# jianwang-mpi/GlobalEgoMocap

Hardware: AMD Instinct MI355X
Metric: optimised windows/sec (10-frame, 15-joint) (higher is better)
Workload: dtype f32

## Files before the change

__graft_entry__.py:

```python
import os
import subprocess
import sys

ROOT = os.path.dirname(os.path.abspath(__file__))
if ROOT not in sys.path:
    sys.path.insert(0, ROOT)

CSRC = os.path.join(ROOT, "globalegomocap_amd", "csrc")
LIB_DIR = os.path.join(ROOT, "globalegomocap_amd", "_lib")
LIB = os.path.join(LIB_DIR, "libgem_hip.so")
SOURCES = ["gem_api.hip", "weights.hip", "stage.hip", "gemm_f32.hip", "gemm_bf16.hip", "decoder_bf16.hip", "energy.hip", "lbfgs.hip", "tail.hip", "tail_bf16.hip", "train.hip", "errors.hip", "chunk_io.hip"]


def _stale():
    if not os.path.exists(LIB):
        return True
    t = os.path.getmtime(LIB)
    deps = [os.path.join(CSRC, f) for f in os.listdir(CSRC)] + [os.path.join(ROOT, "include", "gem_hip.h"),
                                                                os.path.abspath(__file__)]
    return any(os.path.getmtime(d) > t for d in deps)


NO_PACKED_FP32 = ["-Xclang", "-target-feature", "-Xclang", "-packed-fp32-ops", "-DGEM_NO_PACKED_FP32"]
FP_CONTRACT = ["-ffp-contract=on"]
EXTRA_FLAGS = {}
OBJ_DIR = os.path.join(ROOT, "build", "obj")


def _compile_one(args):
    hipcc, src, obj, extra = args
    cmd = [hipcc, "--offload-arch=gfx950", "-O3", "-std=c++17", "-fPIC", "-c", "-Wall", "-Wno-unused-function"] + NO_PACKED_FP32 + FP_CONTRACT + extra + ["-o", obj, src]
    r = subprocess.run(cmd, stderr=subprocess.PIPE, text=True)
    rest = [l for l in r.stderr.splitlines() if "'-packed-fp32-ops' is not a recognized feature for this target" not in l]
    if rest:
        sys.stderr.write("\n".join(rest) + "\n")
    if r.returncode:
        raise subprocess.CalledProcessError(r.returncode, cmd)
    return obj


def _objdump(hipcc=None):
    import shutil
    roots = [os.environ.get("ROCM_PATH", "/opt/rocm")]
    if hipcc:
        roots.insert(0, os.path.dirname(os.path.dirname(os.path.realpath(hipcc))))
    for r in roots:
        c = os.path.join(r, "lib", "llvm", "bin", "llvm-objdump")
        if os.path.exists(c):
            return c
    c = shutil.which("llvm-objdump")
    if c:
        return c
    raise RuntimeError("llvm-objdump not found (looked under %s and on PATH): the build cannot prove the library free of packed "
                       "fp32 arithmetic and refuses to ship it unchecked" % ", ".join(roots))


def device_isa(lib=None, hipcc=None):
    import glob
    import shutil
    import tempfile
    lib = lib or LIB
    objdump = _objdump(hipcc)
    tmp = tempfile.mkdtemp(prefix="gem_isa_")
    try:
        local = os.path.join(tmp, "lib.so")
        shutil.copy(lib, local)
        subprocess.run([objdump, "--offloading", local], check=True, cwd=tmp, stdout=subprocess.DEVNULL, stderr=subprocess.DEVNULL)
        parts = sorted(glob.glob(local + ".*gfx950*"))
        if not parts:
            raise RuntimeError("no gfx950 code object found in %s" % lib)
        return "\n".join(subprocess.run([objdump, "-d", p], check=True, capture_output=True, text=True).stdout for p in parts)
    finally:
        shutil.rmtree(tmp, ignore_errors=True)


def check_no_packed_fp32(lib=None, hipcc=None):
    import re
    isa = device_isa(lib, hipcc)
    bad = re.findall(r"^.*\bv_pk_(?:fma|mul|add)_f32\b.*$", isa, flags=re.M)
    if bad:
        raise RuntimeError("%d packed fp32 VALU instructions in %s (gfx950 hazard beside bf16 MFMAs, DESIGN.md section 4), e.g. %s"
                           % (len(bad), lib or LIB, bad[0].strip()))
    return isa.count("\n")


def build(force=False):
    os.makedirs(LIB_DIR, exist_ok=True)
    if force or _stale():
        from concurrent.futures import ThreadPoolExecutor
        hipcc = os.environ.get("HIPCC", "/opt/rocm/bin/hipcc")
        os.makedirs(OBJ_DIR, exist_ok=True)
        headers = [os.path.join(CSRC, f) for f in os.listdir(CSRC) if f.endswith(".h")] + [os.path.join(ROOT, "include", "gem_hip.h"),
                                                                                             os.path.abspath(__file__)]
        newest_header = max(os.path.getmtime(hd) for hd in headers)
        jobs, objs = [], []
        for s in SOURCES:
            src, obj = os.path.join(CSRC, s), os.path.join(OBJ_DIR, s.replace(".hip", ".o"))
            objs.append(obj)
            if force or not os.path.exists(obj) or os.path.getmtime(obj) < max(os.path.getmtime(src), newest_header):
                jobs.append((hipcc, src, obj, EXTRA_FLAGS.get(s, [])))
        with ThreadPoolExecutor(max_workers=min(6, max(1, len(jobs)))) as pool:
            list(pool.map(_compile_one, jobs))
        tmp_lib = LIB + ".unchecked.%d" % os.getpid()
        try:
            subprocess.run([hipcc, "--offload-arch=gfx950", "-fPIC", "-shared", "-o", tmp_lib] + objs, check=True)
            check_no_packed_fp32(tmp_lib, hipcc)
            os.replace(tmp_lib, LIB)
        finally:
            if os.path.exists(tmp_lib):
                os.remove(tmp_lib)
    import globalegomocap_amd
    from globalegomocap_amd import _capi
    _capi.load_library()


def smoke():
    build()
    import numpy as np
    import torch
    from globalegomocap_amd import synth, vae as vae_schema
    from globalegomocap_amd.camera import FisheyeCamera, DEFAULT_CALIBRATION
    from globalegomocap_amd.engine import WindowEngine, energy_weights, LOCAL_STAGE
    from oracle import np_oracle as O

    torch.cuda.set_device(0)
    shape = vae_schema.VAEShape(latent_dim=64, hidden=(16, 16, 32, 32, 64))
    sd = vae_schema.synthetic_state_dict(shape, seed=3, gain=2.0)
    cam = FisheyeCamera.from_json(DEFAULT_CALIBRATION)
    seq = synth.make_sequence(n_frames=100, seed=4, camera=cam)
    est = np.asarray(seq["estimated_local_skeleton"], dtype=np.float32)
    heat = np.asarray(seq["heatmap_list"], dtype=np.float32)
    starts = np.arange(0, 91, 8, dtype=np.int32)
    nw = len(starts)
    pose = np.stack([est[s:s + 10] for s in starts])
    eng = WindowEngine(shape, cam, max_windows=16)
    eng.load_vae(LOCAL_STAGE, sd)
    mb = eng.mean_bone_length(est)
    rng = np.random.default_rng(0)
    z = rng.normal(size=(nw, shape.latent_dim)).astype(np.float32)
    w = energy_weights(1e-2, 1e-2, 1e-1, 1e-3, 1e-2)
    E, parts, dz, X = eng.energy_grad(LOCAL_STAGE, z, pose, mb, w, heat, starts)
    torch.cuda.synchronize()
    vae = O.fold_vae(sd)
    ocam = O.Camera(poly=np.asarray(cam.poly_w2c), cx=cam.cx, cy=cam.cy)
    ow = O.Weights(1e-2, 1e-2, 1e-1, 1e-3, 1e-2)
    mb_o = O.mean_bone_length(est)
    assert np.allclose(mb.cpu().numpy(), mb_o, rtol=1e-5, atol=1e-6)
    for b in range(nw):
        Xo, acts = O.decode(vae, z[b:b + 1], keep=True)
        f, p, dX = O.energy_and_grad(Xo[0], pose[b], mb_o, ow, ocam, heat[starts[b]:starts[b] + 10])
        dzo = O.decode_backward(vae, dX[None], acts)[0]
        assert np.allclose(X[b].cpu().numpy(), Xo[0], rtol=1e-4, atol=1e-5), "decode mismatch"
        assert abs(float(E[b]) - f) <= 1e-5 * abs(f) + 1e-7, ("energy mismatch", float(E[b]), f)
        assert np.abs(dz[b].cpu().numpy() - dzo).max() <= 1e-3 * np.abs(dzo).max() + 1e-7, "gradient mismatch"
    eps = rng.normal(size=(nw, shape.latent_dim)).astype(np.float32)
    out, stats = eng.optimize_stage(LOCAL_STAGE, pose, mb, eps, w, heat, starts)
    torch.cuda.synchronize()
    st = stats.cpu().numpy()
    assert (st[:, 3] == 1).all(), "a window did not finish"
    trace = eng.read_trace(nw)
    final = np.ascontiguousarray(st[:, 2]).view(np.float32)
    errs, self_errs = [], []
    for b in range(nw):
        X0 = pose[b].astype(np.float32)
        z0 = O.latent_from_pose(vae, X0.reshape(1, 10, 45), eps[b].reshape(1, -1))[0]
        losses = []

        def fun(zz):
            Xd, acts = O.decode(vae, zz[None], keep=True)
            f, _, dX = O.energy_and_grad(Xd[0], X0, mb_o, ow, ocam, heat[starts[b]:starts[b] + 10])
            losses.append(f)
            return f, O.decode_backward(vae, dX[None], acts)[0]
        zo, so = O.lbfgs_strong_wolfe(fun, z0, None)
        ref = O.decode(vae, zo[None])[0]
        n_ref = len(losses)
        zp, _ = O.lbfgs_strong_wolfe(fun, z0 + 1e-6 * np.sign(z0), None)
        self_errs.append(float(np.linalg.norm(O.decode(vae, zp[None])[0] - ref, axis=-1).mean()))
        losses = losses[:n_ref]
# ... 20 lines not shown
```

globalegomocap_amd/csrc/gem_internal.h:

```cpp
#pragma once
#if defined(__HIP_DEVICE_COMPILE__) && !defined(GEM_NO_PACKED_FP32)
#error "compile with: -Xclang -target-feature -Xclang -packed-fp32-ops -DGEM_NO_PACKED_FP32 (__graft_entry__.NO_PACKED_FP32)"
#endif

#include <hip/hip_runtime.h>
#include <stdint.h>
#include <atomic>
#include <set>
#include <string>
#include <vector>

#include "../../include/gem_hip.h"

namespace gem {

constexpr int PAD = 64;
constexpr float LEAKY_SLOPE = 0.01f;
constexpr double BN_EPS = 1e-5;
constexpr int MAX_HIST = 128;
constexpr int MAXJ_ERR = GEM_MAX_JOINTS;
constexpr int N_LOG = 1 << 16;
constexpr int TRACE_ROUNDS = 64;

inline int pad64(int x) { return (x + PAD - 1) / PAD * PAD; }
// ... 172 lines not shown
    v += dpp_move<0xB1>(v);
    v += dpp_move<0x4E>(v);
    v += dpp_move<0x141>(v);
    v += dpp_move<0x140>(v);
    return ((read_lane(v, 0) + read_lane(v, 16)) + read_lane(v, 32)) + read_lane(v, 48);
}
__device__ __forceinline__ double wave_max_dpp(double v) {
    v = nan_max(v, dpp_move<0xB1>(v));
    v = nan_max(v, dpp_move<0x4E>(v));
    v = nan_max(v, dpp_move<0x141>(v));
    v = nan_max(v, dpp_move<0x140>(v));
    return nan_max(nan_max(nan_max(read_lane(v, 0), read_lane(v, 16)), read_lane(v, 32)), read_lane(v, 48));
}

}

namespace gem {
struct GraphKey {
    int kind = 0, stage = 0, B = 0, precision = 0;
    bool tex_cache = true;
    const void* ptr[12] = {};
    gem_energy_weights w[2] = {};
    gem_lbfgs_opts opt = {};
    void* stream = nullptr;
};
struct GraphEntry {
    GraphKey key;
    hipGraph_t graph = nullptr;
    hipGraphExec_t exec = nullptr;
    uint64_t last_use = 0;
};
}

struct gem_handle {
    gem_config cfg;
    int T, J, C, Cp, D, Dp, top, topp;
    gem::StageNet net[2];
    gem::Workspace ws;
    gem::Profile prof;
    int precision = 0;
    int n_cu = 256;
    double* post_work = nullptr;
    size_t post_work_elems = 0;
    bool tex_cache = true;
    bool graphs_on = false;
    std::vector<gem::GraphEntry> graphs;
    uint64_t graph_tick = 0;
    int64_t graph_replays = 0, graph_captures = 0;
    int* d_parents = nullptr;
    int* d_children = nullptr;
};

namespace gem {

void note_kernel(gem_handle* h, const void* host_fn);
inline void commit_kernel_names(gem_handle* h, int family) {
    if (family >= 0 && family < 4) h->prof.names[family].insert(h->prof.pending.begin(), h->prof.pending.end());
    h->prof.pending.clear();
}

int launch_gemm(gem_handle* h, const Layer& L, int epi, const float* A, int lda, const float* aux, float* Cout, int ldc,
                int M, int T, hipStream_t s, int family, const GemmOpts& o = GemmOpts());

int pick_splitk(const gem_handle* h, long blocks, int n_tiles, size_t slab_elems);

struct DynSplit { int RT, SK, per; size_t slab; };
__host__ __device__ inline DynSplit dyn_split(int M, int BM, int CT, int W, int n_tiles, int ldc) {
    DynSplit d;
    d.RT = (M + BM - 1) / BM;
    if (d.RT < 1) d.RT = 1;
    int cap = W / (d.RT * CT);
    if (cap < 1) cap = 1;
    int mx = n_tiles / 4;
    if (mx < 1) mx = 1;
    const int sk = cap < mx ? cap : mx;
    d.per = (n_tiles + sk - 1) / sk;
    d.SK = (n_tiles + d.per - 1) / d.per;
    d.slab = (size_t)d.RT * BM * ldc;
    return d;
}
__device__ inline void slab_layout(const SlabSrc& s, int& nslab, size_t& stride) {
    nslab = s.nslab;
    stride = s.stride;
    if (s.dyn_W > 0) {
        const DynSplit d = dyn_split(*s.m_dev, 64, s.CT, s.dyn_W, s.n_tiles, s.ldc);
        nslab = d.SK;
        stride = d.slab;
    }
}
bool rows_can_fuse_compaction(const gem_handle* h, const Layer& L, int lda, int ldc, int B, bool slabs);
int launch_splitk_reduce(gem_handle* h, int epi, int nslab, size_t slab, const float* bias, const float* aux, float* C, int M, int N,
                         int ldc, const int* m_dev, hipStream_t s, int dyn_W = 0, int n_tiles = 0);
int launch_gemm_bf16(gem_handle* h, const Layer& L, int epi, int nprod, const float* A, int lda, const float* aux, float* Cout,
                     int ldc, int M, int T, hipStream_t s, const GemmOpts& o);

enum Narrow {
    NARROW_BATCHED = 0,
    NARROW_TAIL_F32 = 1,
    NARROW_TAIL_BF16 = 2
};
struct Route {
    int precision = 0;
    Narrow narrow = NARROW_BATCHED;
    bool front = false;
    int tail_wgs = 0;
    int tail_cap = 0;
    Repack repack = REPACK_KERNEL;
};
enum Call { CALL_DECODE = 0, CALL_EVALUATE = 1, CALL_ROUNDS = 2 };
Route plan_route(const gem_handle* h, int stage, int B, Call call);

struct EnergyArgs;
int evaluate_bf16(gem_handle* h, const Route& rt, int stage, int B, const EnergyArgs& ea, hipStream_t s, bool forward_only, const RoundSet* rs,
                  SlabSrc* grad);
int launch_f32_to_bf16(const float* src, uint16_t* dst, size_t n, hipStream_t s);
int launch_f32_split_bf16(const float* src, uint16_t* hi, uint16_t* lo, size_t n, hipStream_t s);

int launch_pack_pose(const float* src, float* dst, int rows, int C, hipStream_t s);
int launch_unpack_pose(const float* src, float* dst, int rows, int C, hipStream_t s);
int launch_reparam(const float* mulv, const float* eps, float* mu, float* logvar, float* z, float* z2, int B, int D, int Dp,
                   hipStream_t s);
int launch_pad_latent(const float* z, float* zp, int B, int D, int Dp, hipStream_t s);
int launch_unpad_latent(const float* zp, float* z, int B, int D, int Dp, hipStream_t s);

struct EnergyArgs {
    const float* Xp;
    const float* X0;
    const float* heat;
    const int32_t* frame0;
    const float* mean_bone;
    float* dXp;
    uint16_t* dXp_b;
    double* f;
    double* parts;
    float w3d, ws, wb, wv, wr;
    double dw3d, dws, dwb, dwv, dwr;
    int T, J, H, W, n_poly;
    float poly[GEM_MAX_POLY];
    float cx, cy;
    const int* parents;
    const int* children;
    int* tex_key;
    float* tex_val;
    const int* n_dev;
    const int* perm;
};
int launch_energy(gem_handle* h, const EnergyArgs& a, int B, hipStream_t s);

constexpr int TAIL_MAX_LAYERS = 6;
struct TailLayerDev { const float* w4; const float* bias; int K, N; };
struct TailArgs {
    int n, B, G, forward_only, escr, mask_first;
    int waves, rows;
    SlabSrc in_slab;
    const float* in_bias;
    int in_bias_ld;
    long long* dbg_ts;
    TailLayerDev fwd[TAIL_MAX_LAYERS], bwd[TAIL_MAX_LAYERS];
    const float* a_in;
    float* g_out;
    uint16_t* g_out_b;
    float* Xp;
    int off_act[TAIL_MAX_LAYERS + 1], ld_act[TAIL_MAX_LAYERS + 1], off_g[2], ld_g, off_red, off_escr, off_zero, off_pre;
    EnergyArgs e;
};
size_t plan_tail(const std::vector<Layer>& dec, int start, int T, int J, TailArgs* out, bool shared = false);
void fill_tail_args(const gem_handle* h, const StageNet& net, const Route& rt, int B, bool forward_only, const SlabSrc& in_slab,
                    const EnergyArgs& ea, const RoundSet* rs, TailArgs* ta);
size_t plan_tail_for(const gem_handle* h, const std::vector<Layer>& dec, int start, int wgs, TailArgs* out);

constexpr int TB_MAX_LAYERS = 6;
struct TailB16Layer { int K, N; const float* bias; };
struct TailB16Args {
    int n, B, G, nrt, forward_only, mask_first;
    SlabSrc in_slab;
    const float* in_bias;
    int in_bias_ld;
    const uint16_t* a_in_b;
    uint16_t* g_out_b;
    float* Xp;
    long long* dbg_ts;
    const uint16_t* wstream;
    int steps_f, steps_total;
    TailB16Layer fwd[TB_MAX_LAYERS], bwd[TB_MAX_LAYERS];
    int off_act[TB_MAX_LAYERS + 1], ld_act[TB_MAX_LAYERS + 1];
    int off_mask[TB_MAX_LAYERS], ld_mask[TB_MAX_LAYERS];
    int off_x, escr, off_mb, off_zero, off_tab;
    int off_bwin, off_epair;
    EnergyArgs e;
};
size_t plan_tail_bf16(const std::vector<Layer>& dec, int start, int T, int J, TailB16Args* out, int nrt = 5);
int tail_bf16_row_tiles(const gem_handle* h, int B, int T);
int build_tail_bf16_stream(gem_handle* h, StageNet& net);
int launch_tail_bf16(gem_handle* h, const TailB16Args& a, size_t lds_bytes, hipStream_t s, const RoundSet* rs = nullptr);
int launch_tail(gem_handle* h, const TailArgs& a, size_t lds_bytes, hipStream_t s, const RoundSet* rs = nullptr);
int tail_cap_workgroups(const gem_handle* h, const std::vector<Layer>& dec, int start);
int launch_mean_bone(gem_handle* h, const float* pose, int n_frames, float* out, hipStream_t s);
int launch_gather_windows(const float* frames, const int32_t* frame0, float* out, int B, int T, int JC, hipStream_t s);
int launch_relative_global(const float* local, const double* cams, const int32_t* frame0, float* rel, int B, int T, int J,
                           hipStream_t s);
int launch_to_global(const float* rel, const double* cams, const int32_t* frame0, double* out, int B, int T, int J,
                     hipStream_t s);

int launch_errors(gem_handle* h, const double* est, const double* mid, const double* opt, const double* gt, int F,
                  const double* bone_mm, double* frame_out, double* out, hipStream_t s, int n_seq);
int launch_merge(const double* win, double* tmp, double* out, int n_chunks, int wpc, int T, int JC, int overlap, int smooth,
                 hipStream_t s);
size_t errors_frame_lds_bytes(int J);
void drop_graphs(gem_handle* h);
int post_scratch(gem_handle* h, size_t elems);
int launch_lift(gem_handle* h, const float* heat, const double* depth, int F, const double* poly, int n_poly, int up, int pad_x,
                int pad_y, double* out64, float* out32, hipStream_t s);

int launch_lbfgs_init(gem_handle* h, int B, hipStream_t s);
int launch_lbfgs_advance(gem_handle* h, int B, const gem_lbfgs_opts& o, const RoundSet& rs, const SlabSrc& grad, hipStream_t s);
int launch_lbfgs_stats(gem_handle* h, int B, gem_window_stats* out, hipStream_t s);
int launch_compact(gem_handle* h, const RoundSet& rs, int B, int force_all, hipStream_t s, int zero_after = 0);
int launch_lbfgs_debug_read(gem_handle* h, int B, gem_lbfgs_debug_state* out, float* x, float* d, float* trial, hipStream_t s);


}
```

globalegomocap_amd/csrc/tail.hip:

```cpp
#include <algorithm>

#include "energy_device.h"

namespace gem {

typedef float f32x16 __attribute__((ext_vector_type(16)));
typedef float f32x4 __attribute__((ext_vector_type(4)));

__device__ __forceinline__ float bf16_round(float x) {
    const __bf16 b = (__bf16)x;
    return (float)b;
}

constexpr int TAIL_WAVES = 8;
constexpr int TAIL_THREADS = TAIL_WAVES * 64;
constexpr int TAIL_WAVES_SHARED = 4;

constexpr int TAIL_ROWS = 16;

template <int W>
__device__ __forceinline__ void tail_prefetch_first(const TailLayerDev L, f32x4 (&dst)[4]) {
    const int lane = threadIdx.x & 63, wave = __builtin_amdgcn_readfirstlane(threadIdx.x >> 6);
    const int c = lane & 15, q = lane >> 4;
    const int n0 = wave * 16;
    if (n0 >= L.N) return;
    const f32x4* p = reinterpret_cast<const f32x4*>(L.w4) + (size_t)q * L.N + n0 + c;
#pragma unroll
    for (int g = 0; g < 4; ++g) dst[g] = p[(size_t)(4 * g) * L.N];
}

template <int W, int NT, typename Epi>
__device__ __forceinline__ void tail_gemm_nt(const float* in, int ld_in, const float* zero_line, const TailLayerDev L,
                                             const TailLayerDev next, bool has_next, int T, int R, f32x4 (&bpre)[4], Epi epi,
                                             int c0 = 0, bool use_pre = true) {
    const int tid = threadIdx.x, lane = tid & 63, wave = __builtin_amdgcn_readfirstlane(tid >> 6);
    const int fr = lane & 15, fq = lane >> 4;
    const int kb = L.K / 64, nblk = 3 * kb;
    const f32x4* W4 = reinterpret_cast<const f32x4*>(L.w4);
    constexpr int TS = 16 * W;
    const int n0 = wave * 16 + c0;
    if (n0 >= L.N) {
        if (has_next) tail_prefetch_first<W>(next, bpre);
        return;
    }
    const int row = fr;
    const int t_row = row % T;
    const bool row_ok = row < R;
    float bv[NT];
    f32x4 acc[NT];
#pragma unroll
    for (int i = 0; i < NT; ++i) {
        bv[i] = L.bias ? L.bias[n0 + TS * i + fr] : 0.f;
        acc[i] = f32x4{0.f, 0.f, 0.f, 0.f};
    }
    const f32x4* pB = W4 + (size_t)fq * L.N + n0 + fr;
    const int strideB = 16 * L.N;
    const int a_own = row * ld_in + 4 * fq;
    const int a_zero = (int)(zero_line - in) + 4 * fq;
    const bool ok_m = row_ok && t_row >= 1, ok_p = row_ok && t_row + 1 < T;
#define TAIL_LOAD_B(blk_, dst_)                                                                        \
    {                                                                                                  \
        const f32x4* p_ = pB + (size_t)(blk_) * strideB;                                               \
        _Pragma("unroll") for (int i = 0; i < NT; ++i)                                                 \
            _Pragma("unroll") for (int g = 0; g < 4; ++g) dst_[i][g] = p_[(size_t)(4 * g) * L.N + TS * i]; \
    }
#define TAIL_LOAD_A(blk_, dst_)                                                                        \
    {                                                                                                  \
        const int tap_ = ((blk_) >= kb) + ((blk_) >= 2 * kb), k0_ = ((blk_) - tap_ * kb) * 64;         \
        const bool ok_ = tap_ == 0 ? ok_m : (tap_ == 1 ? row_ok : ok_p);                               \
        const float* arow_ = in + (ok_ ? a_own + (tap_ - 1) * ld_in + k0_ : a_zero);                   \
        _Pragma("unroll") for (int g = 0; g < 4; ++g) dst_[g] = *reinterpret_cast<const f32x4*>(arow_ + 16 * g); \
    }
#define TAIL_COMPUTE(a_, b_)                                                                           \
    {                                                                                                  \
        _Pragma("unroll") for (int g = 0; g < 4; ++g) {                                                \
            _Pragma("unroll") for (int i = 0; i < NT; ++i) acc[i] = __builtin_amdgcn_mfma_f32_16x16x4f32(a_[g].x, b_[i][g].x, acc[i], 0, 0, 0); \
            _Pragma("unroll") for (int i = 0; i < NT; ++i) acc[i] = __builtin_amdgcn_mfma_f32_16x16x4f32(a_[g].y, b_[i][g].y, acc[i], 0, 0, 0); \
            _Pragma("unroll") for (int i = 0; i < NT; ++i) acc[i] = __builtin_amdgcn_mfma_f32_16x16x4f32(a_[g].z, b_[i][g].z, acc[i], 0, 0, 0); \
            _Pragma("unroll") for (int i = 0; i < NT; ++i) acc[i] = __builtin_amdgcn_mfma_f32_16x16x4f32(a_[g].w, b_[i][g].w, acc[i], 0, 0, 0); \
        }                                                                                              \
    }
    f32x4 b0[NT][4], b1[NT][4], a0[4], a1[4];
    TAIL_LOAD_B(0, b0);
    if (use_pre) {
#pragma unroll
        for (int g = 0; g < 4; ++g) b0[0][g] = bpre[g];
    }
    TAIL_LOAD_A(0, a0);
    const int npairs = nblk / 2;
#define TAIL_INTERLEAVE()                                                                                          \
    {                                                                                                              \
        _Pragma("unroll") for (int i_ = 0; i_ < 4 * NT; ++i_) { __builtin_amdgcn_sched_group_barrier(0x008, 2, 0); __builtin_amdgcn_sched_group_barrier(0x020, 1, 0); } \
        _Pragma("unroll") for (int i_ = 0; i_ < 4; ++i_) { __builtin_amdgcn_sched_group_barrier(0x008, 2 * NT, 0); __builtin_amdgcn_sched_group_barrier(0x100, 1, 0); } \
    }
    for (int p = 0; p < npairs; ++p) {
        const int blk = 2 * p;
        TAIL_LOAD_B(blk + 1, b1);
        TAIL_LOAD_A(blk + 1, a1);
        TAIL_COMPUTE(a0, b0);
        TAIL_INTERLEAVE();
        __builtin_amdgcn_sched_barrier(0);
        const int nxt = min(blk + 2, nblk - 1);
        TAIL_LOAD_B(nxt, b0);
        TAIL_LOAD_A(nxt, a0);
        TAIL_COMPUTE(a1, b1);
        TAIL_INTERLEAVE();
        __builtin_amdgcn_sched_barrier(0);
    }
#undef TAIL_INTERLEAVE
    if (nblk & 1) TAIL_COMPUTE(a0, b0);
    if (has_next) tail_prefetch_first<W>(next, bpre);
#undef TAIL_LOAD_A
#undef TAIL_LOAD_B
#undef TAIL_COMPUTE
#pragma unroll
    for (int i = 0; i < NT; ++i) epi(acc[i], 4 * fq, n0 + TS * i + fr, bv[i]);
}

template <int W, typename Epi>
__device__ __forceinline__ void tail_gemm(const float* in, int ld_in, const float* zero_line, const TailLayerDev L,
                                          const TailLayerDev next, bool has_next, int T, int R, f32x4 (&bpre)[4], Epi epi) {
    if constexpr (W == TAIL_WAVES_SHARED) {
        if (L.N > 32 * W) {
            tail_gemm_nt<W, 2>(in, ld_in, zero_line, L, next, false, T, R, bpre, epi);
            tail_gemm_nt<W, 2>(in, ld_in, zero_line, L, next, has_next, T, R, bpre, epi, 32 * W, false);
        } else if (L.N > 16 * W) tail_gemm_nt<W, 2>(in, ld_in, zero_line, L, next, has_next, T, R, bpre, epi);
        else tail_gemm_nt<W, 1>(in, ld_in, zero_line, L, next, has_next, T, R, bpre, epi);
    } else {
        if (L.N > 32 * W) tail_gemm_nt<W, 4>(in, ld_in, zero_line, L, next, has_next, T, R, bpre, epi);
        else if (L.N > 16 * W) tail_gemm_nt<W, 2>(in, ld_in, zero_line, L, next, has_next, T, R, bpre, epi);
        else tail_gemm_nt<W, 1>(in, ld_in, zero_line, L, next, has_next, T, R, bpre, epi);
    }
}

template <int NL, int W>
__global__ __launch_bounds__(64 * W, W == TAIL_WAVES_SHARED ? 3 : 2) void decoder_tail_kernel(TailArgs a) {
    constexpr int THREADS = 64 * W;
    constexpr bool TIGHT = W == TAIL_WAVES_SHARED;
    constexpr int STAGE_U = 2048 / THREADS;
    constexpr int PRE_E = TAIL_THREADS / THREADS;
    extern __shared__ __attribute__((aligned(16))) float lds[];
    const int tid = threadIdx.x, lane = tid & 63, wave = __builtin_amdgcn_readfirstlane(tid >> 6);
    const int T = a.e.T;
    int probe = 0;
#define TAIL_PROBE()                                                                                   \
    if (a.dbg_ts && blockIdx.x == 0 && tid == 0) {                                                     \
        a.dbg_ts[2 * probe] = clock64();                                                               \
        a.dbg_ts[2 * probe + 1] = wall_clock64();                                                      \
        ++probe;                                                                                       \
    }
    const int w0 = blockIdx.x * a.G;
    const int B = a.e.n_dev ? *a.e.n_dev : a.B;
    if (w0 >= B) return;
    const int nwin = min(a.G, B - w0);
    const int R = nwin * T;
    const size_t row0 = (size_t)w0 * T;

    {
        const int K0 = a.fwd[0].K, q4 = K0 / 4, n4 = (TIGHT ? a.rows : TAIL_ROWS) * q4;
        float* dst = lds + a.off_act[0];
        if (a.in_slab.base) {
            int nslab;
            size_t stride;
            slab_layout(a.in_slab, nslab, stride);
            for (int u = 0; u < STAGE_U; ++u) {
                const int i = tid + u * THREADS, r = i / q4, c = (i - r * q4) * 4;
                if (i >= n4) break;
                f32x4 v = {0.f, 0.f, 0.f, 0.f};
                if (r < R) {
                    const float* p = a.in_slab.base + (row0 + r) * K0 + c;
                    for (int z0 = 0; z0 < nslab; z0 += 8) {
                        f32x4 t[8];
#pragma unroll
                        for (int k = 0; k < 8; ++k) t[k] = *reinterpret_cast<const f32x4*>(p + (size_t)min(z0 + k, nslab - 1) * stride);
#pragma unroll
                        for (int k = 0; k < 8; ++k)
                            if (z0 + k < nslab) v += t[k];
                    }
                    v += *reinterpret_cast<const f32x4*>(a.in_bias + (r % T) * a.in_bias_ld + c);
#pragma unroll
                    for (int q = 0; q < 4; ++q) v[q] = v[q] > 0.f ? v[q] : v[q] * LEAKY_SLOPE;
                }
                *reinterpret_cast<f32x4*>(dst + r * a.ld_act[0] + c) = v;
            }
        } else {
            f32x4 v[STAGE_U];
#pragma unroll
            for (int u = 0; u < STAGE_U; ++u) {
                const int i = tid + u * THREADS, r = i / q4, c = (i - r * q4) * 4;
                v[u] = f32x4{0.f, 0.f, 0.f, 0.f};
                if (i < n4 && r < R) v[u] = *reinterpret_cast<const f32x4*>(a.a_in + (row0 + r) * K0 + c);
            }
#pragma unroll
            for (int u = 0; u < STAGE_U; ++u) {
                const int i = tid + u * THREADS, r = i / q4, c = (i - r * q4) * 4;
                if (i < n4) *reinterpret_cast<f32x4*>(dst + r * a.ld_act[0] + c) = v[u];
            }
        }
        if (tid < 64) lds[a.off_zero + tid] = 0.f;
    }
    float pre_x0[PRE_E], pre_mb = 0.f;
    int pre_par = 0, pre_ch[PRE_E];
#pragma unroll
    for (int k = 0; k < PRE_E; ++k) { pre_x0[k] = 0.f; pre_ch[k] = -1; }
    static_assert(MAXJ * MAXJ <= TAIL_THREADS && MAXJ <= 64, "the children table is parked by PRE_E passes of the workgroup");
    const bool pre_on = a.G == 1 && !a.forward_only && T * a.e.J * 3 <= TAIL_THREADS;
    if (pre_on) {
        const int J = a.e.J, n = T * J * 3, bw = a.e.perm ? a.e.perm[w0] : w0;
#pragma unroll
        for (int k = 0; k < PRE_E; ++k) {
            const int e = tid + k * THREADS;
            if (e < n) pre_x0[k] = a.e.X0[(size_t)bw * n + e];
            if (e < J * MAXJ) pre_ch[k] = a.e.children[e];
        }
        if (tid < J) { pre_mb = a.e.mean_bone[(size_t)bw * J + tid]; pre_par = a.e.parents[tid]; }
    }
    TAIL_PROBE();
    __syncthreads();
    TAIL_PROBE();

    f32x4 bpre[4];
    tail_prefetch_first<W>(a.fwd[0], bpre);
#pragma unroll
    for (int i = 0; i < NL; ++i) {
        const bool last = (i + 1 == NL);
        float* out = lds + a.off_act[i + 1];
        const int ldo = a.ld_act[i + 1];
        float* Xp = last ? a.Xp : nullptr;
        const TailLayerDev nxt = !last ? a.fwd[i + 1 < NL ? i + 1 : i] : a.bwd[NL - 1];
        tail_gemm<W>(lds + a.off_act[i], a.ld_act[i], lds + a.off_zero, a.fwd[i], nxt, !last || !a.forward_only, T, R, bpre,
                  [&](const f32x4& acc, int r0, int col, float bv) {
#pragma unroll
                      for (int e = 0; e < 4; ++e) {
                          float v = acc[e] + bv;
                          if (!last) v = v > 0.f ? v : v * LEAKY_SLOPE;
                          if (!TIGHT || r0 + e < a.rows) out[(r0 + e) * ldo + col] = v;
                          if (Xp && r0 + e < R) Xp[(row0 + r0 + e) * PAD + col] = v;
                      }
                  });
        if (i == 0 && pre_on) {
            const int J = a.e.J, n = T * J * 3;
            float* pre = lds + a.off_pre;
            int* prei = reinterpret_cast<int*>(pre + n + J);
#pragma unroll
            for (int k = 0; k < PRE_E; ++k) {
                const int e = tid + k * THREADS;
                if (e < n) pre[e] = pre_x0[k];
                if (e < J * MAXJ) prei[J + e] = pre_ch[k];
            }
            if (tid < J) { pre[n + tid] = pre_mb; prei[tid] = pre_par; }
        }
        __syncthreads();
        TAIL_PROBE();
    }
    if (a.forward_only) return;

    float* g_cur = lds + a.off_g[0];
    float* g_nxt = lds + a.off_g[1];
    if (a.G == 1) {
        float* scr = lds + a.off_escr;
        const int J = a.e.J, n = T * J * 3;
        const float* pre = lds + a.off_pre;
        const int* prei = reinterpret_cast<const int*>(pre + n + J);
        if (T == 10 && J == 15)
            energy_window<true, THREADS, 10, 15>(a.e, a.e.perm ? a.e.perm[w0] : w0, tid, lds + a.off_act[NL], a.ld_act[NL], scr,
                                                      scr + a.escr, scr + 2 * a.escr, scr + 3 * a.escr, g_cur, a.ld_g, a.fwd[NL - 1].N,
                                                      nullptr, pre_on ? pre : nullptr, pre_on ? pre + n : nullptr, pre_on ? prei : nullptr,
                                                      pre_on ? prei + J : nullptr);
        else
            energy_window<true, THREADS>(a.e, a.e.perm ? a.e.perm[w0] : w0, tid, lds + a.off_act[NL], a.ld_act[NL], scr,
                                              scr + a.escr, scr + 2 * a.escr, scr + 3 * a.escr, g_cur, a.ld_g, a.fwd[NL - 1].N,
                                              nullptr, pre_on ? pre : nullptr, pre_on ? pre + n : nullptr, pre_on ? prei : nullptr,
                                              pre_on ? prei + J : nullptr);
    } else if (wave < nwin) {
        float* scr = lds + a.off_escr + wave * 4 * a.escr;
        energy_window<false>(a.e, a.e.perm ? a.e.perm[w0 + wave] : w0 + wave, lane,
                             lds + a.off_act[NL] + wave * T * a.ld_act[NL], a.ld_act[NL], scr, scr + a.escr,
                             scr + 2 * a.escr, scr + 3 * a.escr, g_cur + wave * T * a.ld_g, a.ld_g, a.fwd[NL - 1].N);
    }
    __syncthreads();
    TAIL_PROBE();

#pragma unroll
    for (int i = NL - 1; i >= 0; --i) {
        const float* act = lds + a.off_act[i];
        const int lda = a.ld_act[i];
        const int ldg = a.ld_g;
        float* gout = a.g_out;
        uint16_t* gout_b = a.g_out_b;
        const int K0 = a.fwd[0].K;
        tail_gemm<W>(g_cur, a.ld_g, lds + a.off_zero, a.bwd[i], a.bwd[i > 0 ? i - 1 : 0], i > 0, T, R, bpre,
                  [&](const f32x4& acc, int r0, int col, float) {
#pragma unroll
                      for (int e = 0; e < 4; ++e) {
                          const int row = r0 + e;
                          const float v = (i > 0 || a.mask_first) ? acc[e] * (act[row * lda + col] > 0.f ? 1.f : LEAKY_SLOPE) : acc[e];
                          if (i > 0) { if (!TIGHT || row < a.rows) g_nxt[row * ldg + col] = v; }
                          else if (row < R) {
                              if (gout_b) gout_b[(row0 + row) * K0 + col] = (uint16_t)(__builtin_bit_cast(unsigned int, bf16_round(v)) >> 16);
                              else gout[(row0 + row) * K0 + col] = v;
                          }
                      }
                  });
        __syncthreads();
        TAIL_PROBE();
        float* t = g_cur; g_cur = g_nxt; g_nxt = t;
    }
#undef TAIL_PROBE
}

size_t plan_tail(const std::vector<Layer>& dec, int start, int T, int J, TailArgs* out, bool shared) {
    const int n = (int)dec.size() - start;
    if (start < 0 || n < 1 || n > TAIL_MAX_LAYERS || T > TAIL_ROWS) return 0;
    for (int i = start; i < (int)dec.size(); ++i) {
        const int K = dec[i].K, N = dec[i].N;
        auto ok = [](int v) { return v == 64 || v == 128 || v == 256 || v == 512; };
        if (!ok(K) || !ok(N)) return 0;
    }
    TailArgs a{};
    a.n = n;
    a.mask_first = start > 0;
    a.G = TAIL_ROWS / T;
    if (shared && a.G != 1) return 0;
    a.waves = shared ? TAIL_WAVES_SHARED : TAIL_WAVES;
    a.rows = shared ? a.G * T : TAIL_ROWS;
    const int rows = a.rows;
    int off = 0, maxg = 0;
    for (int i = 0; i <= n; ++i) {
        const int width = i == 0 ? dec[start].K : dec[start + i - 1].N;
        a.off_act[i] = off;
        a.ld_act[i] = width + 4;
        off += rows * (width + 4);
        if (i >= 1 && width > maxg) maxg = width;
    }
    a.ld_g = maxg + 4;
    a.off_g[0] = off; off += rows * a.ld_g;
    a.off_g[1] = off; off += rows * a.ld_g;
    a.escr = (T * J * 3 + 3) / 4 * 4;
    a.off_red = off;
    a.off_escr = off;
    off += a.G * 4 * a.escr;
    a.off_zero = off;
    off += 64;
    a.off_pre = off;
    if (a.G == 1) off += (T * J * 3 + 2 * J + J * MAXJ + 3) / 4 * 4;
    if (out) *out = a;
    return (size_t)off * sizeof(float);
}

template <int NL, int W>
static void launch_tail_as(gem_handle* h, const TailArgs& a, int wgs, size_t lds_bytes, hipStream_t s) {
    note_kernel(h, reinterpret_cast<const void*>(decoder_tail_kernel<NL, W>));
    hipLaunchKernelGGL((decoder_tail_kernel<NL, W>), dim3(wgs), dim3(64 * W), lds_bytes, s, a);
}

template <int W>
static int launch_tail_w(gem_handle* h, const TailArgs& a, int wgs, size_t lds_bytes, hipStream_t s) {
    switch (a.n) {
        case 1: launch_tail_as<1, W>(h, a, wgs, lds_bytes, s); break;
        case 2: launch_tail_as<2, W>(h, a, wgs, lds_bytes, s); break;
        case 3: launch_tail_as<3, W>(h, a, wgs, lds_bytes, s); break;
        case 4: launch_tail_as<4, W>(h, a, wgs, lds_bytes, s); break;
        case 5: launch_tail_as<5, W>(h, a, wgs, lds_bytes, s); break;
        case 6: launch_tail_as<6, W>(h, a, wgs, lds_bytes, s); break;
        default: set_error("launch_tail: unsupported number of fused layers"); return 1;
    }
    return 0;
}

static bool tail_can_share_cu(const std::vector<Layer>& dec, int start, int T, int J) {
    const size_t bytes = plan_tail(dec, start, T, J, nullptr, true);
    if (!bytes || 3 * bytes > 160 * 1024) return false;
    for (int i = start; i < (int)dec.size(); ++i)
        if (dec[i].N > 64 * TAIL_WAVES_SHARED || dec[i].K > 64 * TAIL_WAVES_SHARED) return false;
    return true;
}

size_t plan_tail_for(const gem_handle* h, const std::vector<Layer>& dec, int start, int wgs, TailArgs* out) {
    bool shared = wgs > h->n_cu && tail_can_share_cu(dec, start, h->T, h->J);
    if (const char* f = dev_env("GEM_TAIL_WAVES")) shared = atoi(f) == TAIL_WAVES_SHARED && tail_can_share_cu(dec, start, h->T, h->J);
    return plan_tail(dec, start, h->T, h->J, out, shared);
}

int tail_cap_workgroups(const gem_handle* h, const std::vector<Layer>& dec, int start) {
    if (const char* f = dev_env("GEM_TAIL_CAP")) return atoi(f) * h->n_cu;
    return (tail_can_share_cu(dec, start, h->T, h->J) ? 10 : 5) * h->n_cu;
}

int launch_tail(gem_handle* h, const TailArgs& a, size_t lds_bytes, hipStream_t s, const RoundSet* rs) {
    static PerDeviceOnce attr_once;
    if (attr_once.need(h->cfg.device)) {
        const void* ks[] = {reinterpret_cast<const void*>(decoder_tail_kernel<1, 8>), reinterpret_cast<const void*>(decoder_tail_kernel<2, 8>),
                            reinterpret_cast<const void*>(decoder_tail_kernel<3, 8>), reinterpret_cast<const void*>(decoder_tail_kernel<4, 8>),
                            reinterpret_cast<const void*>(decoder_tail_kernel<5, 8>), reinterpret_cast<const void*>(decoder_tail_kernel<6, 8>),
                            reinterpret_cast<const void*>(decoder_tail_kernel<1, 4>), reinterpret_cast<const void*>(decoder_tail_kernel<2, 4>),
                            reinterpret_cast<const void*>(decoder_tail_kernel<3, 4>), reinterpret_cast<const void*>(decoder_tail_kernel<4, 4>),
                            reinterpret_cast<const void*>(decoder_tail_kernel<5, 4>), reinterpret_cast<const void*>(decoder_tail_kernel<6, 4>)};
        for (const void* k : ks) GEM_HIP(hipFuncSetAttribute(k, hipFuncAttributeMaxDynamicSharedMemorySize, 160 * 1024));
    }
    Profile::Rec rec;
    const bool prof = h->prof.on;
    if (prof) {
        GEM_HIP(hipEventCreate(&rec.a)); GEM_HIP(hipEventCreate(&rec.b));
        rec.family = 1;
        double per_window = 0.0;
        for (int i = 0; i < a.n; ++i) per_window += 2.0 * 3.0 * a.fwd[i].K * a.fwd[i].N * a.e.T;
        if (!a.forward_only) per_window *= 2.0;
        rec.flops = per_window * a.B;
        if (rs) { rec.log_idx = rs->log_idx; rec.flops_per_window = per_window; }
        GEM_HIP(hipEventRecord(rec.a, s));
    }
    const int wgs = (a.B + a.G - 1) / a.G;
    if (a.waves != TAIL_WAVES && a.waves != TAIL_WAVES_SHARED) { set_error("launch_tail: the arguments do not come from plan_tail"); return 1; }
    if (a.waves == TAIL_WAVES_SHARED ? launch_tail_w<TAIL_WAVES_SHARED>(h, a, wgs, lds_bytes, s) : launch_tail_w<TAIL_WAVES>(h, a, wgs, lds_bytes, s))
        return 1;
    GEM_HIP(hipGetLastError());
    if (prof) { GEM_HIP(hipEventRecord(rec.b, s)); h->prof.recs.push_back(rec); }
    commit_kernel_names(h, prof ? 1 : -1);
    return 0;
}

}
```

Before: 32070.

## Deepen tail GEMM weight prefetch with register ring and early next-layer prefetch

The fused decoder-tail GEMM's two-buffer ping-pong becomes a configurable register ring. When the tail layers are narrow (at most two column tiles), the kernel prefetches the next layer's B blocks and bias for every tile before computing the current layer, so those global loads overlap the current MFMA work. Kernels are now also specialised on the widest layer, so narrow networks drop the four-tile path and its register pressure, and a higher unroll threshold is set for tail.hip. The cost is more live registers and more code paths, which can lower occupancy or cause spills.

```diff
diff --git a/__graft_entry__.py b/__graft_entry__.py
--- a/__graft_entry__.py
+++ b/__graft_entry__.py
@@ -23,7 +23,7 @@
 
 NO_PACKED_FP32 = ["-Xclang", "-target-feature", "-Xclang", "-packed-fp32-ops", "-DGEM_NO_PACKED_FP32"]
 FP_CONTRACT = ["-ffp-contract=on"]
-EXTRA_FLAGS = {}
+EXTRA_FLAGS = {"tail.hip": ["-mllvm", "-pragma-unroll-threshold=65536"]}
 OBJ_DIR = os.path.join(ROOT, "build", "obj")
 
 
diff --git a/globalegomocap_amd/csrc/gem_internal.h b/globalegomocap_amd/csrc/gem_internal.h
--- a/globalegomocap_amd/csrc/gem_internal.h
+++ b/globalegomocap_amd/csrc/gem_internal.h
@@ -348,6 +348,7 @@
 struct TailArgs {
     int n, B, G, forward_only, escr, mask_first;
     int waves, rows;
+    int maxnt;
     SlabSrc in_slab;
     const float* in_bias;
     int in_bias_ld;
diff --git a/globalegomocap_amd/csrc/tail.hip b/globalegomocap_amd/csrc/tail.hip
--- a/globalegomocap_amd/csrc/tail.hip
+++ b/globalegomocap_amd/csrc/tail.hip
@@ -18,21 +18,68 @@
 
 constexpr int TAIL_ROWS = 16;
 
-template <int W>
-__device__ __forceinline__ void tail_prefetch_first(const TailLayerDev L, f32x4 (&dst)[4]) {
+#ifndef TAIL_PREFETCH_BLOCKS
+#define TAIL_PREFETCH_BLOCKS 1
+#endif
+#ifndef TAIL_RING_DEPTH
+#define TAIL_RING_DEPTH 2
+#endif
+#ifndef TAIL_PREFETCH_EARLY
+#define TAIL_PREFETCH_EARLY 1
+#endif
+template <int W, int MAXNT>
+struct TailSched {
+    static constexpr bool DEEP = W == TAIL_WAVES && MAXNT <= 2;
+    static constexpr int P = DEEP ? TAIL_PREFETCH_BLOCKS : 1;
+    static constexpr int D = DEEP ? TAIL_RING_DEPTH : 2;
+    static constexpr int NTP = DEEP ? MAXNT : 1;
+    static constexpr int PW = P < D - 1 ? P : D - 1;
+    static constexpr bool EARLY = DEEP && TAIL_PREFETCH_EARLY;
+    static_assert(P >= 1 && D >= 2 && D <= 4, "ring of two to four register sets");
+};
+template <int W, int MAXNT>
+struct TailPre {
+    f32x4 b[TailSched<W, MAXNT>::P][4];
+    f32x4 bx[TailSched<W, MAXNT>::NTP > 1 ? TailSched<W, MAXNT>::NTP - 1 : 1][TailSched<W, MAXNT>::PW][4];
+    float bias[TailSched<W, MAXNT>::NTP];
+};
+
+template <int W, int MAXNT>
+__device__ __forceinline__ void tail_prefetch(const TailLayerDev L, TailPre<W, MAXNT>& dst) {
+    using S = TailSched<W, MAXNT>;
     const int lane = threadIdx.x & 63, wave = __builtin_amdgcn_readfirstlane(threadIdx.x >> 6);
     const int c = lane & 15, q = lane >> 4;
     const int n0 = wave * 16;
     if (n0 >= L.N) return;
-    const f32x4* p = reinterpret_cast<const f32x4*>(L.w4) + (size_t)q * L.N + n0 + c;
-#pragma unroll
-    for (int g = 0; g < 4; ++g) dst[g] = p[(size_t)(4 * g) * L.N];
-}
-
-template <int W, int NT, typename Epi>
+    const int nblk = 3 * (L.K / 64);
+    const int nb = nblk <= S::P ? nblk : S::PW;
+    const char* p = reinterpret_cast<const char*>(reinterpret_cast<const f32x4*>(L.w4) + n0);
+    const unsigned vo = (unsigned)(q * L.N + c) * 16u;
+#pragma unroll
+    for (int i = 0; i < S::NTP; ++i) {
+        if (n0 + 16 * W * i < L.N) {
+#pragma unroll
+            for (int s = 0; s < (i == 0 ? S::P : S::PW); ++s) {
+                if (s < nb) {
+#pragma unroll
+                    for (int g = 0; g < 4; ++g) {
+                        const f32x4 v = *reinterpret_cast<const f32x4*>(p + (((size_t)16 * s + 4 * g) * L.N + 16 * W * i) * 16 + vo);
+                        if (i == 0) dst.b[s][g] = v;
+                        else dst.bx[i > 0 ? i - 1 : 0][s][g] = v;
+                    }
+                }
+            }
+            if constexpr (S::DEEP) dst.bias[i] = L.bias ? L.bias[n0 + 16 * W * i + c] : 0.f;
+        }
+    }
+}
+
+template <int W, int MAXNT, int NT, typename Epi>
 __device__ __forceinline__ void tail_gemm_nt(const float* in, int ld_in, const float* zero_line, const TailLayerDev L,
-                                             const TailLayerDev next, bool has_next, int T, int R, f32x4 (&bpre)[4], Epi epi,
+                                             const TailLayerDev next, bool has_next, int T, int R, TailPre<W, MAXNT>& pre, Epi epi,
                                              int c0 = 0, bool use_pre = true) {
+    using S = TailSched<W, MAXNT>;
+    constexpr int P = S::P, D = S::D, NTP = S::NTP, PW = S::PW;
     const int tid = threadIdx.x, lane = tid & 63, wave = __builtin_amdgcn_readfirstlane(tid >> 6);
     const int fr = lane & 15, fq = lane >> 4;
     const int kb = L.K / 64, nblk = 3 * kb;
@@ -40,7 +87,7 @@
     constexpr int TS = 16 * W;
     const int n0 = wave * 16 + c0;
     if (n0 >= L.N) {
-        if (has_next) tail_prefetch_first<W>(next, bpre);
+        if (has_next) tail_prefetch<W, MAXNT>(next, pre);
         return;
     }
     const int row = fr;
@@ -50,20 +97,23 @@
     f32x4 acc[NT];
 #pragma unroll
     for (int i = 0; i < NT; ++i) {
-        bv[i] = L.bias ? L.bias[n0 + TS * i + fr] : 0.f;
+        if (S::DEEP && i < NTP && use_pre) bv[i] = pre.bias[i];
+        else bv[i] = L.bias ? L.bias[n0 + TS * i + fr] : 0.f;
         acc[i] = f32x4{0.f, 0.f, 0.f, 0.f};
     }
-    const f32x4* pB = W4 + (size_t)fq * L.N + n0 + fr;
+    const char* pB = reinterpret_cast<const char*>(W4 + n0);
+    const unsigned vB = (unsigned)(fq * L.N + fr) * 16u;
     const int strideB = 16 * L.N;
     const int a_own = row * ld_in + 4 * fq;
     const int a_zero = (int)(zero_line - in) + 4 * fq;
     const bool ok_m = row_ok && t_row >= 1, ok_p = row_ok && t_row + 1 < T;
+#define TAIL_LOAD_B1(blk_, dst_, i_)                                                                   \
+    {                                                                                                  \
+        const char* p_ = pB + ((size_t)(blk_) * strideB + TS * (i_)) * 16;                             \
+        _Pragma("unroll") for (int g = 0; g < 4; ++g) dst_[i_][g] = *reinterpret_cast<const f32x4*>(p_ + (size_t)(64 * g) * L.N + vB); \
+    }
 #define TAIL_LOAD_B(blk_, dst_)                                                                        \
-    {                                                                                                  \
-        const f32x4* p_ = pB + (size_t)(blk_) * strideB;                                               \
-        _Pragma("unroll") for (int i = 0; i < NT; ++i)                                                 \
-            _Pragma("unroll") for (int g = 0; g < 4; ++g) dst_[i][g] = p_[(size_t)(4 * g) * L.N + TS * i]; \
-    }
+    { _Pragma("unroll") for (int i = 0; i < NT; ++i) TAIL_LOAD_B1(blk_, dst_, i); }
 #define TAIL_LOAD_A(blk_, dst_)                                                                        \
     {                                                                                                  \
         const int tap_ = ((blk_) >= kb) + ((blk_) >= 2 * kb), k0_ = ((blk_) - tap_ * kb) * 64;         \
@@ -80,61 +130,106 @@
             _Pragma("unroll") for (int i = 0; i < NT; ++i) acc[i] = __builtin_amdgcn_mfma_f32_16x16x4f32(a_[g].w, b_[i][g].w, acc[i], 0, 0, 0); \
         }                                                                                              \
     }
-    f32x4 b0[NT][4], b1[NT][4], a0[4], a1[4];
-    TAIL_LOAD_B(0, b0);
-    if (use_pre) {
-#pragma unroll
-        for (int g = 0; g < 4; ++g) b0[0][g] = bpre[g];
-    }
-    TAIL_LOAD_A(0, a0);
-    const int npairs = nblk / 2;
-#define TAIL_INTERLEAVE()                                                                                          \
+#define TAIL_INTERLEAVE(LB_)                                                                                       \
     {                                                                                                              \
-        _Pragma("unroll") for (int i_ = 0; i_ < 4 * NT; ++i_) { __builtin_amdgcn_sched_group_barrier(0x008, 2, 0); __builtin_amdgcn_sched_group_barrier(0x020, 1, 0); } \
+        if (LB_) { _Pragma("unroll") for (int i_ = 0; i_ < 4 * NT; ++i_) { __builtin_amdgcn_sched_group_barrier(0x008, 2, 0); __builtin_amdgcn_sched_group_barrier(0x020, 1, 0); } } \
+        else __builtin_amdgcn_sched_group_barrier(0x008, 8 * NT, 0);                                               \
         _Pragma("unroll") for (int i_ = 0; i_ < 4; ++i_) { __builtin_amdgcn_sched_group_barrier(0x008, 2 * NT, 0); __builtin_amdgcn_sched_group_barrier(0x100, 1, 0); } \
     }
-    for (int p = 0; p < npairs; ++p) {
-        const int blk = 2 * p;
-        TAIL_LOAD_B(blk + 1, b1);
-        TAIL_LOAD_A(blk + 1, a1);
-        TAIL_COMPUTE(a0, b0);
-        TAIL_INTERLEAVE();
-        __builtin_amdgcn_sched_barrier(0);
-        const int nxt = min(blk + 2, nblk - 1);
-        TAIL_LOAD_B(nxt, b0);
-        TAIL_LOAD_A(nxt, a0);
-        TAIL_COMPUTE(a1, b1);
-        TAIL_INTERLEAVE();
-        __builtin_amdgcn_sched_barrier(0);
-    }
+#define TAIL_STEP(blk_, s_, LB_, bcur_)                                                                \
+    {                                                                                                  \
+        if (LB_) TAIL_LOAD_B((blk_) + D - 1, b[((s_) + D - 1) % D]);                                   \
+        TAIL_LOAD_A(min((blk_) + 1, nblk - 1), a[((s_) + 1) % D]);                                     \
+        TAIL_COMPUTE(a[(s_) % D], bcur_);                                                              \
+        TAIL_INTERLEAVE(LB_);                                                                          \
+        __builtin_amdgcn_sched_barrier(0);                                                             \
+    }
+    f32x4 a[D][4], b[D][NT][4];
+    TailPre<W, MAXNT> pre_next;
+    bool whole = false;
+    if constexpr (P >= 3 && NT == 1) whole = use_pre && nblk <= P;
+    if constexpr (S::EARLY) {
+        if (use_pre) {
+#pragma unroll
+            for (int s = 0; s < P; ++s) {
+                if (s < PW || whole) {
+#pragma unroll
+                    for (int g = 0; g < 4; ++g) asm volatile("" : "+v"(pre.b[s][g]));
+                }
+            }
+#pragma unroll
+            for (int i = 1; i < (NT < NTP ? NT : NTP); ++i)
+#pragma unroll
+                for (int s = 0; s < PW; ++s)
+#pragma unroll
+                    for (int g = 0; g < 4; ++g) asm volatile("" : "+v"(pre.bx[i - 1][s][g]));
+        }
+        if (has_next) tail_prefetch<W, MAXNT>(next, pre_next);
+    }
+    TAIL_LOAD_A(0, a[0]);
+    if (whole) {
+        if constexpr (P >= 3 && NT == 1) {
+            static_assert(P == 3, "a layer has at least three blocks: K = 64, three taps");
+#pragma unroll
+            for (int t = 0; t < P; ++t) TAIL_STEP(t, t, false, (&pre.b[t]));
+        }
+    } else {
+#pragma unroll
+        for (int s = 0; s < D - 1; ++s)
+#pragma unroll
+            for (int i = 0; i < NT; ++i) {
+                if (s < PW && i < NTP && use_pre) {
+#pragma unroll
+                    for (int g = 0; g < 4; ++g) b[s][i][g] = i == 0 ? pre.b[s][g] : pre.bx[i > 0 ? i - 1 : 0][s < PW ? s : 0][g];
+                } else TAIL_LOAD_B1(s, b[s], i);
+            }
+        const int nl = nblk - (D - 1), ngrp = nl / D, r = nl - ngrp * D;
+        for (int grp = 0; grp < ngrp; ++grp) {
+#pragma unroll
+            for (int j = 0; j < D; ++j) TAIL_STEP(grp * D + j, j, true, b[j]);
+        }
+        const int blk0 = ngrp * D;
+#pragma unroll
+        for (int rr = 0; rr < D; ++rr) {
+            if (r != rr) continue;
+#pragma unroll
+            for (int t = 0; t < rr + D - 1; ++t) TAIL_STEP(blk0 + t, t, t < rr, b[t % D]);
+        }
+    }
+    if constexpr (S::EARLY) pre = pre_next;
+    else if (has_next) tail_prefetch<W, MAXNT>(next, pre);
+#undef TAIL_STEP
 #undef TAIL_INTERLEAVE
-    if (nblk & 1) TAIL_COMPUTE(a0, b0);
-    if (has_next) tail_prefetch_first<W>(next, bpre);
 #undef TAIL_LOAD_A
 #undef TAIL_LOAD_B
+#undef TAIL_LOAD_B1
 #undef TAIL_COMPUTE
 #pragma unroll
     for (int i = 0; i < NT; ++i) epi(acc[i], 4 * fq, n0 + TS * i + fr, bv[i]);
 }
 
-template <int W, typename Epi>
+template <int W, int MAXNT, typename Epi>
 __device__ __forceinline__ void tail_gemm(const float* in, int ld_in, const float* zero_line, const TailLayerDev L,
-                                          const TailLayerDev next, bool has_next, int T, int R, f32x4 (&bpre)[4], Epi epi) {
+                                          const TailLayerDev next, bool has_next, int T, int R, TailPre<W, MAXNT>& pre, Epi epi) {
     if constexpr (W == TAIL_WAVES_SHARED) {
         if (L.N > 32 * W) {
-            tail_gemm_nt<W, 2>(in, ld_in, zero_line, L, next, false, T, R, bpre, epi);
-            tail_gemm_nt<W, 2>(in, ld_in, zero_line, L, next, has_next, T, R, bpre, epi, 32 * W, false);
-        } else if (L.N > 16 * W) tail_gemm_nt<W, 2>(in, ld_in, zero_line, L, next, has_next, T, R, bpre, epi);
-        else tail_gemm_nt<W, 1>(in, ld_in, zero_line, L, next, has_next, T, R, bpre, epi);
+            tail_gemm_nt<W, MAXNT, 2>(in, ld_in, zero_line, L, next, false, T, R, pre, epi);
+            tail_gemm_nt<W, MAXNT, 2>(in, ld_in, zero_line, L, next, has_next, T, R, pre, epi, 32 * W, false);
+        } else if (L.N > 16 * W) tail_gemm_nt<W, MAXNT, 2>(in, ld_in, zero_line, L, next, has_next, T, R, pre, epi);
+        else tail_gemm_nt<W, MAXNT, 1>(in, ld_in, zero_line, L, next, has_next, T, R, pre, epi);
     } else {
-        if (L.N > 32 * W) tail_gemm_nt<W, 4>(in, ld_in, zero_line, L, next, has_next, T, R, bpre, epi);
-        else if (L.N > 16 * W) tail_gemm_nt<W, 2>(in, ld_in, zero_line, L, next, has_next, T, R, bpre, epi);
-        else tail_gemm_nt<W, 1>(in, ld_in, zero_line, L, next, has_next, T, R, bpre, epi);
-    }
-}
-
+        if constexpr (MAXNT >= 4) {
+            if (L.N > 32 * W) { tail_gemm_nt<W, MAXNT, 4>(in, ld_in, zero_line, L, next, has_next, T, R, pre, epi); return; }
+        }
+        if (L.N > 16 * W) tail_gemm_nt<W, MAXNT, 2>(in, ld_in, zero_line, L, next, has_next, T, R, pre, epi);
+        else tail_gemm_nt<W, MAXNT, 1>(in, ld_in, zero_line, L, next, has_next, T, R, pre, epi);
+    }
+}
+
+template <int MAXNT>
+struct TailTiles {
 template <int NL, int W>
-__global__ __launch_bounds__(64 * W, W == TAIL_WAVES_SHARED ? 3 : 2) void decoder_tail_kernel(TailArgs a) {
+static __global__ __launch_bounds__(64 * W, W == TAIL_WAVES_SHARED ? 3 : 2) void decoder_tail_kernel(TailArgs a) {
     constexpr int THREADS = 64 * W;
     constexpr bool TIGHT = W == TAIL_WAVES_SHARED;
     constexpr int STAGE_U = 2048 / THREADS;
@@ -219,8 +314,8 @@
     __syncthreads();
     TAIL_PROBE();
 
-    f32x4 bpre[4];
-    tail_prefetch_first<W>(a.fwd[0], bpre);
+    TailPre<W, MAXNT> bpre;
+    tail_prefetch<W, MAXNT>(a.fwd[0], bpre);
 #pragma unroll
     for (int i = 0; i < NL; ++i) {
         const bool last = (i + 1 == NL);
@@ -228,7 +323,7 @@
         const int ldo = a.ld_act[i + 1];
         float* Xp = last ? a.Xp : nullptr;
         const TailLayerDev nxt = !last ? a.fwd[i + 1 < NL ? i + 1 : i] : a.bwd[NL - 1];
-        tail_gemm<W>(lds + a.off_act[i], a.ld_act[i], lds + a.off_zero, a.fwd[i], nxt, !last || !a.forward_only, T, R, bpre,
+        tail_gemm<W, MAXNT>(lds + a.off_act[i], a.ld_act[i], lds + a.off_zero, a.fwd[i], nxt, !last || !a.forward_only, T, R, bpre,
                   [&](const f32x4& acc, int r0, int col, float bv) {
 #pragma unroll
                       for (int e = 0; e < 4; ++e) {
@@ -289,7 +384,7 @@
         float* gout = a.g_out;
         uint16_t* gout_b = a.g_out_b;
         const int K0 = a.fwd[0].K;
-        tail_gemm<W>(g_cur, a.ld_g, lds + a.off_zero, a.bwd[i], a.bwd[i > 0 ? i - 1 : 0], i > 0, T, R, bpre,
+        tail_gemm<W, MAXNT>(g_cur, a.ld_g, lds + a.off_zero, a.bwd[i], a.bwd[i > 0 ? i - 1 : 0], i > 0, T, R, bpre,
                   [&](const f32x4& acc, int r0, int col, float) {
 #pragma unroll
                       for (int e = 0; e < 4; ++e) {
@@ -308,6 +403,7 @@
     }
 #undef TAIL_PROBE
 }
+};
 
 size_t plan_tail(const std::vector<Layer>& dec, int start, int T, int J, TailArgs* out, bool shared) {
     const int n = (int)dec.size() - start;
@@ -324,6 +420,9 @@
     if (shared && a.G != 1) return 0;
     a.waves = shared ? TAIL_WAVES_SHARED : TAIL_WAVES;
     a.rows = shared ? a.G * T : TAIL_ROWS;
+    int widest = 0;
+    for (int i = start; i < (int)dec.size(); ++i) widest = std::max(widest, std::max(dec[i].K, dec[i].N));
+    a.maxnt = !shared && widest > 32 * TAIL_WAVES ? 4 : 2;
     const int rows = a.rows;
     int off = 0, maxg = 0;
     for (int i = 0; i <= n; ++i) {
@@ -348,21 +447,21 @@
     return (size_t)off * sizeof(float);
 }
 
-template <int NL, int W>
+template <int NL, int W, int MAXNT>
 static void launch_tail_as(gem_handle* h, const TailArgs& a, int wgs, size_t lds_bytes, hipStream_t s) {
-    note_kernel(h, reinterpret_cast<const void*>(decoder_tail_kernel<NL, W>));
-    hipLaunchKernelGGL((decoder_tail_kernel<NL, W>), dim3(wgs), dim3(64 * W), lds_bytes, s, a);
-}
-
-template <int W>
+    note_kernel(h, reinterpret_cast<const void*>(&TailTiles<MAXNT>::template decoder_tail_kernel<NL, W>));
+    hipLaunchKernelGGL((TailTiles<MAXNT>::template decoder_tail_kernel<NL, W>), dim3(wgs), dim3(64 * W), lds_bytes, s, a);
+}
+
+template <int W, int MAXNT>
 static int launch_tail_w(gem_handle* h, const TailArgs& a, int wgs, size_t lds_bytes, hipStream_t s) {
     switch (a.n) {
-        case 1: launch_tail_as<1, W>(h, a, wgs, lds_bytes, s); break;
-        case 2: launch_tail_as<2, W>(h, a, wgs, lds_bytes, s); break;
-        case 3: launch_tail_as<3, W>(h, a, wgs, lds_bytes, s); break;
-        case 4: launch_tail_as<4, W>(h, a, wgs, lds_bytes, s); break;
-        case 5: launch_tail_as<5, W>(h, a, wgs, lds_bytes, s); break;
-        case 6: launch_tail_as<6, W>(h, a, wgs, lds_bytes, s); break;
+        case 1: launch_tail_as<1, W, MAXNT>(h, a, wgs, lds_bytes, s); break;
+        case 2: launch_tail_as<2, W, MAXNT>(h, a, wgs, lds_bytes, s); break;
+        case 3: launch_tail_as<3, W, MAXNT>(h, a, wgs, lds_bytes, s); break;
+        case 4: launch_tail_as<4, W, MAXNT>(h, a, wgs, lds_bytes, s); break;
+        case 5: launch_tail_as<5, W, MAXNT>(h, a, wgs, lds_bytes, s); break;
+        case 6: launch_tail_as<6, W, MAXNT>(h, a, wgs, lds_bytes, s); break;
         default: set_error("launch_tail: unsupported number of fused layers"); return 1;
     }
     return 0;
@@ -390,12 +489,15 @@
 int launch_tail(gem_handle* h, const TailArgs& a, size_t lds_bytes, hipStream_t s, const RoundSet* rs) {
     static PerDeviceOnce attr_once;
     if (attr_once.need(h->cfg.device)) {
-        const void* ks[] = {reinterpret_cast<const void*>(decoder_tail_kernel<1, 8>), reinterpret_cast<const void*>(decoder_tail_kernel<2, 8>),
-                            reinterpret_cast<const void*>(decoder_tail_kernel<3, 8>), reinterpret_cast<const void*>(decoder_tail_kernel<4, 8>),
-                            reinterpret_cast<const void*>(decoder_tail_kernel<5, 8>), reinterpret_cast<const void*>(decoder_tail_kernel<6, 8>),
-                            reinterpret_cast<const void*>(decoder_tail_kernel<1, 4>), reinterpret_cast<const void*>(decoder_tail_kernel<2, 4>),
-                            reinterpret_cast<const void*>(decoder_tail_kernel<3, 4>), reinterpret_cast<const void*>(decoder_tail_kernel<4, 4>),
-                            reinterpret_cast<const void*>(decoder_tail_kernel<5, 4>), reinterpret_cast<const void*>(decoder_tail_kernel<6, 4>)};
+        const void* ks[] = {reinterpret_cast<const void*>(&TailTiles<2>::decoder_tail_kernel<1, 8>), reinterpret_cast<const void*>(&TailTiles<2>::decoder_tail_kernel<2, 8>),
+                            reinterpret_cast<const void*>(&TailTiles<2>::decoder_tail_kernel<3, 8>), reinterpret_cast<const void*>(&TailTiles<2>::decoder_tail_kernel<4, 8>),
+                            reinterpret_cast<const void*>(&TailTiles<2>::decoder_tail_kernel<5, 8>), reinterpret_cast<const void*>(&TailTiles<2>::decoder_tail_kernel<6, 8>),
+                            reinterpret_cast<const void*>(&TailTiles<4>::decoder_tail_kernel<1, 8>), reinterpret_cast<const void*>(&TailTiles<4>::decoder_tail_kernel<2, 8>),
+                            reinterpret_cast<const void*>(&TailTiles<4>::decoder_tail_kernel<3, 8>), reinterpret_cast<const void*>(&TailTiles<4>::decoder_tail_kernel<4, 8>),
+                            reinterpret_cast<const void*>(&TailTiles<4>::decoder_tail_kernel<5, 8>), reinterpret_cast<const void*>(&TailTiles<4>::decoder_tail_kernel<6, 8>),
+                            reinterpret_cast<const void*>(&TailTiles<2>::decoder_tail_kernel<1, 4>), reinterpret_cast<const void*>(&TailTiles<2>::decoder_tail_kernel<2, 4>),
+                            reinterpret_cast<const void*>(&TailTiles<2>::decoder_tail_kernel<3, 4>), reinterpret_cast<const void*>(&TailTiles<2>::decoder_tail_kernel<4, 4>),
+                            reinterpret_cast<const void*>(&TailTiles<2>::decoder_tail_kernel<5, 4>), reinterpret_cast<const void*>(&TailTiles<2>::decoder_tail_kernel<6, 4>)};
         for (const void* k : ks) GEM_HIP(hipFuncSetAttribute(k, hipFuncAttributeMaxDynamicSharedMemorySize, 160 * 1024));
     }
     Profile::Rec rec;
@@ -411,9 +513,14 @@
         GEM_HIP(hipEventRecord(rec.a, s));
     }
     const int wgs = (a.B + a.G - 1) / a.G;
-    if (a.waves != TAIL_WAVES && a.waves != TAIL_WAVES_SHARED) { set_error("launch_tail: the arguments do not come from plan_tail"); return 1; }
-    if (a.waves == TAIL_WAVES_SHARED ? launch_tail_w<TAIL_WAVES_SHARED>(h, a, wgs, lds_bytes, s) : launch_tail_w<TAIL_WAVES>(h, a, wgs, lds_bytes, s))
-        return 1;
+    bool planned = (a.waves == TAIL_WAVES && (a.maxnt == 2 || a.maxnt == 4)) || (a.waves == TAIL_WAVES_SHARED && a.maxnt == 2);
+    for (int i = 0; planned && i < a.n && i < TAIL_MAX_LAYERS; ++i)
+        planned = std::max(a.fwd[i].N, a.bwd[i].N) <= (a.waves == TAIL_WAVES ? 16 * TAIL_WAVES * a.maxnt : 64 * TAIL_WAVES_SHARED);
+    if (!planned) { set_error("launch_tail: the arguments do not come from plan_tail"); return 1; }
+    const int err = a.waves == TAIL_WAVES_SHARED ? launch_tail_w<TAIL_WAVES_SHARED, 2>(h, a, wgs, lds_bytes, s)
+                    : a.maxnt == 4           ? launch_tail_w<TAIL_WAVES, 4>(h, a, wgs, lds_bytes, s)
+                                             : launch_tail_w<TAIL_WAVES, 2>(h, a, wgs, lds_bytes, s);
+    if (err) return 1;
     GEM_HIP(hipGetLastError());
     if (prof) { GEM_HIP(hipEventRecord(rec.b, s)); h->prof.recs.push_back(rec); }
     commit_kernel_names(h, prof ? 1 : -1);
```

Result: faster. 32480, median of 6 (+1.3%).
